# spotify/basic-pitch

Hardware: NVIDIA H100
Metric: audio_seconds_per_second (higher is better)
Workload: dtype f32

## Files before the change

basic_pitch_b200/_lib.py:

```python
from __future__ import annotations

import ctypes as C
import os
import pathlib
from typing import Optional

LIB_PATH = pathlib.Path(__file__).resolve().parent / "libbp_b200.so"

BP_OK = 0
BP_E_INVALID = -1
BP_E_CUDA = -2
BP_E_CAPACITY = -3
BP_E_NOMEM = -4

EXPORTS = [
    "bp_version", "bp_last_error", "bp_default_decode_params", "bp_num_windows", "bp_num_frames",
    "bp_model_create", "bp_model_destroy", "bp_model_device", "bp_model_param_block", "bp_model_refresh",
    "bp_model_launch_count", "bp_forward_device", "bp_forward_host", "bp_run_inference_device",
    "bp_run_inference_host", "bp_decode_device", "bp_decode_host", "bp_transcribe_host", "bp_transcribe_device",
    "bp_infer_onsets_host", "bp_pitch_bends_host", "bp_debug_activation", "bp_model_chunk_windows", "bp_model_set_path", "bp_model_profile", "bp_model_profile_read", "bp_debug_tc_plan", "bp_debug_tc_gather", "bp_debug_tc_gather_packed", "bp_debug_tc_b2", "bp_debug_tc_clocks", "bp_transcribe_files_host", "bp_host_alloc", "bp_host_free", "bp_last_required", "bp_resampled_length", "bp_load_pcm_device", "bp_load_pcm_host", "bp_debug_resample_filter", "bp_write_note_files", "bp_sonify_notes_host", "bp_load_pcm_files_device", "bp_transcribe_pcm_files_host", "bp_debug_pcm_layout", "bp_debug_frontend", "bp_model_set_debug_frontend", "bp_debug_chain_layout", "bp_debug_split_layout", "bp_decode_grid_device", "bp_decode_grid_host", "bp_decode_grid_chunk_params", "bp_default_score_params", "bp_frame_times", "bp_score_grid_device", "bp_score_grid_host", "bp_score_notes_host", "bp_multipitch_map", "bp_score_frames_grid_device", "bp_score_frames_grid_host", "bp_score_multipitch_host", "bp_score_salience_grid_device", "bp_score_salience_grid_host", "bp_score_salience_chunk_params", "bp_match_grid_device", "bp_match_grid_host", "bp_match_notes_host", "bp_score_onset_offset_grid_device", "bp_score_onset_offset_grid_host", "bp_score_onset_offset_notes_host",
]


class DecodeParams(C.Structure):
    _fields_ = [
        ("onset_thresh", C.c_double),
        ("frame_thresh", C.c_double),
        ("min_note_len", C.c_int32),
        ("energy_tol", C.c_int32),
        ("infer_onsets", C.c_int32),
        ("melodia_trick", C.c_int32),
        ("include_pitch_bends", C.c_int32),
        ("min_pitch_idx", C.c_int32),
        ("max_pitch_idx", C.c_int32),
        ("reserved", C.c_int32),
    ]


class Notes(C.Structure):
    _fields_ = [
        ("note_capacity", C.c_int32),
        ("bend_capacity", C.c_int32),
        ("note_off", C.c_void_p),
        ("start_frame", C.c_void_p),
        ("end_frame", C.c_void_p),
        ("pitch_midi", C.c_void_p),
        ("amplitude", C.c_void_p),
        ("bend_off", C.c_void_p),
        ("bends", C.c_void_p),
    ]


class NoteSet(C.Structure):
# ... 109 lines not shown
    lib.bp_match_notes_host.argtypes = [vp, C.POINTER(NoteSet), C.POINTER(NoteSet), i32, C.POINTER(ScoreParams), vp]
    lib.bp_score_onset_offset_grid_device.argtypes = [vp, vp, vp, vp, i32, C.POINTER(DecodeParams), i32,
                                                      C.POINTER(NoteSet), C.POINTER(ScoreParams), vp, vp, vp]
    lib.bp_score_onset_offset_grid_host.argtypes = [vp, vp, vp, vp, i32, C.POINTER(DecodeParams), i32,
                                                    C.POINTER(NoteSet), C.POINTER(ScoreParams), vp, vp]
    lib.bp_score_onset_offset_notes_host.argtypes = [vp, C.POINTER(NoteSet), C.POINTER(NoteSet), i32,
                                                     C.POINTER(ScoreParams), vp]
    lib.bp_multipitch_map.argtypes = [vp, i64, vp, i64, vp]
    lib.bp_score_frames_grid_device.argtypes = [vp, vp, vp, vp, i32, C.POINTER(DecodeParams), i32, C.POINTER(MultipitchSet),
                                                C.c_double, vp, vp, vp, vp]
    lib.bp_score_frames_grid_host.argtypes = [vp, vp, vp, vp, i32, C.POINTER(DecodeParams), i32, C.POINTER(MultipitchSet),
                                              C.c_double, vp, vp, vp]
    lib.bp_score_multipitch_host.argtypes = [vp, C.POINTER(MultipitchSet), C.POINTER(MultipitchSet), i32, C.c_double, vp]
    lib.bp_score_salience_grid_device.argtypes = [vp, vp, i32, vp, i32, C.POINTER(SalienceParams), i32,
                                                  C.POINTER(MultipitchSet), C.c_double, vp, vp, vp, vp]
    lib.bp_score_salience_grid_host.argtypes = [vp, vp, i32, vp, i32, C.POINTER(SalienceParams), i32,
                                                C.POINTER(MultipitchSet), C.c_double, vp, vp, vp]
    lib.bp_score_salience_chunk_params.argtypes = [i64, i64]
    lib.bp_score_salience_chunk_params.restype = i64
    lib.bp_transcribe_host.argtypes = [vp, vp, vp, i32, C.POINTER(DecodeParams), vp, vp, vp, vp, C.POINTER(Notes)]
    lib.bp_transcribe_device.argtypes = [vp, vp, vp, i32, C.POINTER(DecodeParams), vp, C.POINTER(Notes), vp]
    lib.bp_infer_onsets_host.argtypes = [vp, vp, vp, i64, vp]
    lib.bp_pitch_bends_host.argtypes = [vp, vp, i64, i32, vp, vp, vp, vp, vp, i64]
    lib.bp_debug_activation.argtypes = [vp, C.c_int, vp, i64]
    lib.bp_debug_frontend.argtypes = [vp, C.c_int, vp, i64]
    lib.bp_model_set_debug_frontend.argtypes = [vp, C.c_int]
    lib.bp_debug_chain_layout.argtypes = [vp, vp, vp]
    lib.bp_debug_split_layout.argtypes = [vp, vp]
    lib.bp_debug_tc_plan.argtypes = [C.c_int, vp, vp, vp, vp, vp, vp, vp]
    lib.bp_debug_tc_gather.argtypes = [C.c_int, vp, vp, vp, vp, vp]
    lib.bp_debug_tc_gather_packed.argtypes = [C.c_int, vp, vp, vp, vp]
    lib.bp_debug_tc_b2.argtypes = [C.c_int, vp, vp, vp]
    lib.bp_debug_tc_clocks.argtypes = [vp, C.c_int, vp, C.c_int]
    lib.bp_transcribe_files_host.argtypes = [vp, vp, vp, i32, C.POINTER(DecodeParams), vp, vp, vp, vp, C.POINTER(Notes)]
    lib.bp_host_alloc.argtypes = [sz]
    lib.bp_host_alloc.restype = vp
    lib.bp_host_free.argtypes = [vp]
    lib.bp_host_free.restype = None
    lib.bp_last_required.argtypes = [vp, vp]
    lib.bp_last_required.restype = None
    lib.bp_resampled_length.argtypes = [i64, i32]
    lib.bp_resampled_length.restype = i64
    lib.bp_load_pcm_device.argtypes = [vp, vp, i32, i64, i32, i32, vp, vp]
    lib.bp_load_pcm_host.argtypes = [vp, vp, i32, i64, i32, i32, vp]
    lib.bp_load_pcm_files_device.argtypes = [vp, C.POINTER(PcmFile), i32, vp, vp, vp]
    lib.bp_transcribe_pcm_files_host.argtypes = [vp, C.POINTER(PcmFile), i32, C.POINTER(DecodeParams), vp, vp, vp, vp, vp,
                                                 C.POINTER(Notes)]
    lib.bp_debug_pcm_layout.argtypes = [C.POINTER(PcmFile), i32, vp, vp]
    lib.bp_debug_resample_filter.argtypes = [i32, i32, vp, i64]
    lib.bp_debug_resample_filter.restype = i64
    lib.bp_write_note_files.argtypes = [i32, vp, vp, vp, vp, vp, vp, vp, vp, vp, i32, C.c_double, i32]
    lib.bp_sonify_notes_host.argtypes = [vp, i32, vp, vp, vp, vp, vp, vp, vp, i32, i32, vp, vp, i64]
    lib.bp_model_profile.argtypes = [vp, C.c_int]
    lib.bp_model_profile_read.argtypes = [vp, C.POINTER(C.c_double), C.POINTER(i64), C.POINTER(i64)]
    for name in EXPORTS:
        fn = getattr(lib, name)
        if fn.restype is C.c_int and name not in ("bp_version", "bp_model_device"):
            fn.errcheck = _check
    _lib = lib
    return lib


def _check(result, func, args):
    if result != BP_OK:
        raise BpError(result, load().bp_last_error().decode(errors="replace"))
    return result
# ... 1 lines not shown
```

basic_pitch_b200/csrc/api.cu:

```cuda
#include <cuda_runtime.h>

#include <algorithm>
#include <atomic>
#include <chrono>
#include <climits>
#include <cmath>
#include <cstdio>
#include <cstring>
#include <memory>
#include <thread>
#include <string>
#include <vector>

#include "bp_b200.h"
#include "kernels.cuh"

using namespace bp;

namespace {

thread_local std::string g_err;

int fail(int code, const std::string& msg) {
  g_err = msg;
// ... 2865 lines not shown
  sizes[0] = g.K_packed;
  if (b1) {
    std::vector<uint16_t> m;
    tc_build_b1(which, w, m);
    std::memcpy(b1, m.data(), m.size() * 2);
  }
  if (kmap) std::copy(g.kmap.begin(), g.kmap.end(), kmap);
  return BP_OK;
}

int bp_debug_tc_b2(int which, const float* w2, int32_t* sizes, uint16_t* tiles) {
  if (!w2 || !sizes || which < 0 || which > 2) return fail(BP_E_INVALID, "bp_debug_tc_b2: bad argument");
  std::vector<uint16_t> t;
  tc_build_b2(which, w2, t);
  const TcConvSpec sp = tc_spec(which);
  sizes[0] = sp.n2_tiles;
  sizes[1] = sp.n2;
  sizes[2] = sp.KH2;
  sizes[3] = sp.width;
  sizes[4] = sp.js;
  if (tiles) std::memcpy(tiles, t.data(), t.size() * 2);
  return BP_OK;
}

int bp_debug_tc_clocks(bp_model_t* m, int which, uint64_t* cycles, int reset) {
  if (!m || !cycles || which < 0 || which > 2) return fail(BP_E_INVALID, "bp_debug_tc_clocks: bad argument");
  DeviceGuard g(m->device);
  CK(cudaDeviceSynchronize());
  if (tc_read_clocks(which, reinterpret_cast<unsigned long long*>(cycles), reset != 0) != 0)
    return fail(BP_E_INVALID, "bp_debug_tc_clocks: the library was built without -DBP_TC_CLOCKS");
  return BP_OK;
}

int bp_model_profile(bp_model_t* m, int which) {
  if (!m) return fail(BP_E_INVALID, "bp_model_profile: null model");
  if (which < -1 || which > 6) return fail(BP_E_INVALID, "bp_model_profile: unknown kernel family");
  m->profile_which = which;
  m->prof_used = 0;
  m->prof_windows = 0;
  return BP_OK;
}

int bp_model_profile_read(bp_model_t* m, double* total_ms, int64_t* n_intervals, int64_t* n_windows) {
  if (!m || !total_ms || !n_intervals || !n_windows) return fail(BP_E_INVALID, "bp_model_profile_read: null argument");
  DeviceGuard g(m->device);
  CK(cudaDeviceSynchronize());
  double total = 0.0;
  for (size_t i = 0; i + 1 < m->prof_used; i += 2) {
    float ms = 0.f;
    CK(cudaEventElapsedTime(&ms, m->prof_ev[i], m->prof_ev[i + 1]));
    total += ms;
  }
  *total_ms = total;
  *n_intervals = (int64_t)(m->prof_used / 2);
  *n_windows = m->prof_windows;
  return BP_OK;
}

int bp_debug_activation(bp_model_t* m, int which, float* h_out, int64_t n_windows) {
  if (!m || !h_out) return fail(BP_E_INVALID, "bp_debug_activation: null argument");
  if (n_windows <= 0 || n_windows > m->chunk || n_windows > m->last_forward_n)
    return fail(BP_E_INVALID, "bp_debug_activation: only valid for the windows of a single-chunk forward call");
  DeviceGuard g(m->device);
  const float* src = nullptr;
  size_t per = 0;
  switch (which) {
// ... 101 lines not shown
```

basic_pitch_b200/csrc/kernels.cuh:

```cuda
#pragma once
#include <cuda_bf16.h>

#include <cstring>
#include <vector>

#include "common.cuh"

namespace bp {

void hcqt_setup();
constexpr int kLp2 = kTaps + 14;
struct Lowpass2 {
  float2 t[kLp2];
};
Lowpass2 lowpass_pairs(const float* h_lp );
void launch_decimate(const Lowpass2& lp, const float* audio, const WinDesc* desc, float* chain, int stage, int n_windows,
                     cudaStream_t st);
void launch_cqt(const float* audio, const WinDesc* desc, const float* chain, const float* wt, const float* scale,
                float* logmag, unsigned int* minmax, int n_windows, cudaStream_t st);
void launch_lognorm(float* y, const unsigned int* minmax, const float* bn , int n_windows,
                    cudaStream_t st);

struct CnnWeights {
  const float *contour1_wT, *contour1_b;
// ... 22 lines not shown
  int layer;
  int KH2, HALO, G0;
  int PD;
  int n2_tiles, n2, js, width, pass;
  int W;
  int slot[24];
  __host__ __device__ constexpr int n_ft() const { return (WOUT + FLT - 1) / FLT; }
  __host__ __device__ constexpr int tile_bins() const { return 8 * (chunks8 - 1); }
  __host__ __device__ constexpr int ksteps() const { return (KH * n_ci * W + 15) / 16; }
  __host__ __device__ constexpr int edge_per_side() const { return 2 * HALO + (layer == 0 ? 8 - HALO : 0); }
};
__host__ __device__ constexpr TcConvSpec tc_spec(int layer) {
  return layer == 0 ? TcConvSpec{3, 39, 1, 1, 19, 8, 16, 264, 8, {-36, 0, 36, 57, 72, 84, 93, 101}, kCqtBins,     40, 174, 3, 0, 5, 2, 9,  1,  1, 32, 5, 104, 40, 0, {}}
       : layer == 1 ? TcConvSpec{5, 5, 3, 2, 1, 32, 4, 88, 8, {-36, 0, 36, 57, 72, 84, 93, 101},   kCqtBins,     40, 174, 3, 1, 3, 1, 12, 12, 2, 16, 4, 32, 32,   6,
                                 {9, 10, 21, 22, 14, 4, 2, 1, 16, 3, 6, 13, 5, 17, 18, 20, 19, 23, 7, 0, 8, 15, 12, 11}}
                    : TcConvSpec{7, 7, 3, 3, 2, 32, 4, 88, 1, {0, 0, 0, 0, 0, 0, 0, 0},           kContourBins, 34, 175, 6, 2, 7, 1, 12, 12, 2, 32, 8, 64, 64,   8, {}};
}
__host__ __device__ constexpr int tc_group_tile(const TcConvSpec& s, int g, int slot) {
  if (g < 0 || g >= s.G0) return -1;
  const int run = g / s.PD, i = g - run * s.PD, ft = 2 * s.PD * run + slot * s.PD + i;
  return ft < s.n_ft() ? ft : -1;
}
__host__ __device__ constexpr int tc_tile_group(const TcConvSpec& s, int ft) {
  const int run = ft / (2 * s.PD), r = ft - run * 2 * s.PD, slot = r / s.PD;
  return ((run * s.PD + r - slot * s.PD) << 1) | slot;
}
__host__ __device__ constexpr bool tc_starts_range(const TcConvSpec& s, int g, int slot, bool item_start) {
  const int ft = tc_group_tile(s, g, slot);
  return item_start || ft <= 0 || tc_group_tile(s, g - 1, slot) != ft - 1;
}
__host__ __device__ constexpr bool tc_ends_range(const TcConvSpec& s, int g, int slot, bool item_end) {
  return item_end || tc_group_tile(s, g + 1, slot) != tc_group_tile(s, g, slot) + 1;
}
__host__ __device__ constexpr bool tc_item_starts(const TcConvSpec& s, int n_split, int g) {
  const int q = (g * n_split + s.G0 - 1) / s.G0;
  return q < n_split && q * s.G0 / n_split == g;
}
__host__ __device__ constexpr bool tc_pairing_ok(const TcConvSpec& s) {
  for (int ft = 0; ft < s.n_ft(); ++ft) {
    int n = 0;
    for (int g = 0; g < s.G0; ++g)
      for (int slot = 0; slot < 2; ++slot) n += tc_group_tile(s, g, slot) == ft;
    const int gs = tc_tile_group(s, ft);
    if (n != 1 || tc_group_tile(s, gs >> 1, gs & 1) != ft) return false;
  }
  return true;
}
struct TcConvPlan {
  TcConvSpec spec{};
  std::vector<uint16_t> tiles;
  std::vector<int> tile_seq;
  std::vector<uint32_t> slot_words[2];
  std::vector<int> group_step_off;
  std::vector<int> group_ft;
  int n_tiles = 0, n_groups = 0, n_uses = 0;
  void build(const TcConvSpec& spec, const float* w );
};
struct TcConvDev {
  int layer;
  const uint16_t* tiles;
  const uint16_t* b1;
  const uint16_t* b2;
  float bias1[32];
  float bias2;
  float note_w[9];
};
int tc_upload_program(const TcConvPlan& contour_plan, cudaStream_t st);
void tc_build_b1(int layer, const float* w, std::vector<uint16_t>& out, bool window8 = false);
struct TcGatherGeom {
  int K, n_ci, KH, wout;
  int K_packed;
  std::vector<int> starts, ranges;
  std::vector<int> kmap;
};
TcGatherGeom tc_gather_geometry(int layer);
void tc_build_b2(int layer, const float* w2, std::vector<uint16_t>& out);
void tc_build_b2_full(int layer, const float* w2, std::vector<uint16_t>& out);
int tc_rows_total(int n_windows, int rows_per_window);
size_t tc_edge_floats(const TcConvSpec& spec, int n_windows);
int tc_setup();
int tc_read_clocks(int layer, unsigned long long* out, bool reset);
struct UnwrapDesc {
  long long dst_base;
  int rows;
  int pad;
};
void launch_lognorm_split(const float* y, const unsigned int* minmax, const float* bn, __nv_bfloat16* dst,
                          const TcConvSpec& spec, int n_windows, int rows_stride, cudaStream_t st);
struct TcOut {
  float* raw = nullptr;
  float* unwrapped = nullptr;
  long long frame_stride = 0;
  long long raw_rows = 0;
  const UnwrapDesc* ud = nullptr;
  const float* note_raw = nullptr;
  __nv_bfloat16* chl = nullptr;
  int chl_rows = 0, chl_chunks = 0, chl_rpw = 0, chl_lead = 0;
  float* edge = nullptr;
  float* act = nullptr;
};
void launch_conv_tc(const __nv_bfloat16* data, const TcConvDev& dev, const TcOut& out, int n_windows, int rows_stride,
                    int n_sms, cudaStream_t st, bool fuse_next = false);
void launch_contour2_tc(const float* c1_nhwc, const CnnWeights& w, float* contour, __nv_bfloat16* chl, int rows_total,
                        int n_windows, cudaStream_t st);

void build_cqt_tc_weights(const float* cqt_real, const float* cqt_imag, std::vector<uint16_t>& out);
void cqt_tc_setup();
void launch_cqt_tc(const float* audio, const WinDesc* desc, const float* chain, const uint16_t* wtc, const float* scale,
                   float* logmag, unsigned int* minmax, int n_windows, int n_sms, cudaStream_t st);

void launch_rows_to_pm(const float* rows, long long n_frames, int width, float* pm, long long stride, long long dst_frame0,
                       cudaStream_t st, const UnwrapDesc* ud = nullptr, int n_windows = 0);
void launch_rows_to_cm(const float* rows, long long n_frames, float* cm, long long stride, long long dst_frame0,
                       cudaStream_t st, const UnwrapDesc* ud = nullptr, int n_windows = 0);
void launch_pm_to_rows(const float* pm, long long stride, long long src_frame0, long long n_frames, int width, float* rows,
                       cudaStream_t st);
void launch_cm_to_rows(const float* cm, long long stride, long long src_frame0, long long n_frames, float* rows,
                       cudaStream_t st);

long long ingest_output_length(long long n_frames, int sample_rate);
std::vector<double> ingest_filter(int up, int down);
int launch_ingest(int device, const void* d_pcm, int format, long long n_frames, int channels, int sample_rate, float* d_out,
                  cudaStream_t st);
struct IngestFile {
  const void* pcm;
  const float* hp;
  float* out;
  long long n_in, n_out;
  int channels, format, up, down, half, taps, span, pad;
};
int ingest_geometry(int format, int channels, int sample_rate, IngestFile& f);
int ingest_taps(int device, IngestFile& f);
long long ingest_ctas(long long n_out);
int launch_ingest_batch(const IngestFile* d_files, const int* d_cta_off, int n_files, int n_ctas, int max_span,
                        cudaStream_t st);
// ... 143 lines not shown
```

basic_pitch_b200/csrc/tc_conv.cu:

```cuda
#include <cuda.h>
#include <cuda_bf16.h>

#include <algorithm>
#include <cstdlib>
#include <cstring>
#include <unordered_map>
#include <vector>

#include "kernels.cuh"
#include "tc_ptx.cuh"

namespace bp {

namespace tc {
constexpr int kMTile = 64;
constexpr int kTileBytes = 8192;
constexpr int kMaxSteps = 1024;
constexpr int kMaxGroups = 15;
static_assert(tc_spec(0).G0 <= kMaxGroups, "contour groups in constant memory");
static_assert(tc_pairing_ok(tc_spec(0)) && tc_pairing_ok(tc_spec(1)) && tc_pairing_ok(tc_spec(2)), "group -> tile map");
static_assert(tc_spec(0).n_ft() <= 2 * tc_spec(0).G0 && tc_spec(1).n_ft() <= 2 * tc_spec(1).G0 &&
                  tc_spec(2).n_ft() <= 2 * tc_spec(2).G0,
              "every tile has a place in the reference pairing of the summation order (TcConvPlan::build)");
constexpr int kConsumerWarps = 8;
// ... 377 lines not shown
      const float* p = y + ((size_t)b * kFrames + t) * kCqtBins;
      float raw[2][8];
#pragma unroll
      for (int h = 0; h < 2; ++h)
#pragma unroll
        for (int j = 0; j < 8; ++j) {
          const int bin = (qa + h * half) * 8 + j;
          raw[h][j] = bin < kCqtBins ? __ldg(p + bin) : 0.f;
        }
#pragma unroll
      for (int h = 0; h < 2; ++h)
#pragma unroll
        for (int j = 0; j < 8; ++j)
          if ((qa + h * half) * 8 + j < kCqtBins) {
            const float q = (mx == 0.f) ? 0.f : __fdiv_rn(__fsub_rn(raw[h][j], mn), mx);
            v[h][j] = __fadd_rn(__fmul_rn(q, bn_scale), bn_bias);
          }
    }
  }
  const size_t plane = (size_t)chunks8 * rows_total * 8;
  store_split8(v[0], dst, ((size_t)qa * rows_total + d) * 8, plane);
  store_split8(v[1], dst, ((size_t)(qa + half) * rows_total + d) * 8, plane);
}

struct TcArgs {
  CUtensorMap data_map;
  int use_tmap;
  const __nv_bfloat16* data;
  const uint16_t* tiles;
  const uint16_t* b1;
  const uint16_t* b2;
  TcOut o;
  int edge_rows;
  int rows_total, n_mtiles, n_windows;
  int n_split;
  int row0;
  int chunks8;
  int ms, h2;
  float bias1[32], bias2, note_w[9];
};

__device__ __forceinline__ float sigmoidf_fast(float x) { return __fdividef(1.f, 1.f + __expf(-x)); }

namespace tc {
enum TcClk {
  kClkFull,
  kClkMma,
  kClkEpi,
  kClkData,
  kClkConsOther,
  kClkEmpty,
  kClkDataEmpty,
  kClkProdOther,
  kNumClk
};
}
#ifdef BP_TC_CLOCKS
__device__ unsigned long long g_tc_clocks[3][tc::kNumClk];
struct TcClocks {
  uint32_t t, c[tc::kNumClk];
  __device__ __forceinline__ TcClocks() {
    t = (uint32_t)clock();
#pragma unroll
    for (int k = 0; k < tc::kNumClk; ++k) c[k] = 0;
  }
  __device__ __forceinline__ void lap(int k) {
    const uint32_t n = (uint32_t)clock();
    c[k] += n - t;
    t = n;
  }
  __device__ __forceinline__ void flush(int layer) {
    if ((threadIdx.x & 31) == 0)
#pragma unroll
      for (int k = 0; k < tc::kNumClk; ++k) atomicAdd(&g_tc_clocks[layer][k], (unsigned long long)c[k]);
  }
};
#else
struct TcClocks {
  __device__ __forceinline__ void lap(int) {}
  __device__ __forceinline__ void flush(int) {}
};
#endif

int tc_read_clocks(int layer, unsigned long long* out, bool reset) {
#ifdef BP_TC_CLOCKS
  if (layer < 0 || layer > 2) return -1;
  if (cudaMemcpyFromSymbol(out, g_tc_clocks, tc::kNumClk * sizeof(unsigned long long),
                           (size_t)layer * tc::kNumClk * sizeof(unsigned long long)) != cudaSuccess)
    return -1;
  if (reset) {
    static const unsigned long long zero[tc::kNumClk] = {};
    if (cudaMemcpyToSymbol(g_tc_clocks, zero, sizeof(zero), (size_t)layer * sizeof(zero)) != cudaSuccess) return -1;
  }
  return 0;
#else
  (void)layer, (void)out, (void)reset;
  return -1;
#endif
}

__device__ __forceinline__ void slot_barrier(int slot) {
  asm volatile("bar.sync %0, 128;" ::"r"(1 + slot) : "memory");
}


struct RowOut {
  float* raw;
  float* unw;
  __nv_bfloat16* chl;
  float* edge;
  const float* note_col;
  int t;
  bool ok;
};

// ... 261 lines not shown
  unsigned char* s_data = smem;
  unsigned char* s_w = smem + SM.data_bytes;
  unsigned char* s_b1 = s_w + kStages * kTileBytes;
  unsigned char* s_b2 = s_b1 + SM.b1_bytes;
  float* s_p = reinterpret_cast<float*>(s_b2 + SM.b2_bytes);
  uint64_t* bars = reinterpret_cast<uint64_t*>(reinterpret_cast<unsigned char*>(s_p) + SM.p_bytes);
  uint64_t* full_w = bars;
  uint64_t* empty_w = bars + kStages;
  uint64_t* data_full = bars + 2 * kStages;
  uint64_t* data_empty = data_full + 1;
  uint64_t* b2_full = data_empty + 1;
  uint64_t* b1_full = b2_full + 1;
  uint32_t* issued = reinterpret_cast<uint32_t*>(b1_full + 1);

  const int warp = __shfl_sync(0xffffffffu, (int)(threadIdx.x >> 5), 0);
  const int lane = threadIdx.x & 31;
  constexpr uint32_t lbo = kDataRows * 16u;
  constexpr uint32_t plane_bytes = (L.chunks8 - 1) * lbo;

  if (threadIdx.x == 0) {
    for (int s = 0; s < kStages; ++s) {
      mbar_init(full_w + s, 1);
      mbar_init(empty_w + s, kConsumerWarps);
    }
    mbar_init(data_full, 1);
    mbar_init(data_empty, kConsumerWarps);
    mbar_init(b2_full, 1);
    mbar_init(b1_full, 1);
    *issued = 0;
    asm volatile("fence.mbarrier_init.release.cluster;" ::: "memory");
  }
  __syncthreads();

  const int n_items = a.n_mtiles * a.n_split;
  TcClocks clk;

  if (warp >= kConsumerWarps) {
    setmaxnreg_dec<kProducerRegs>();
    if (warp != kProducerWarp) return;
    const uint32_t leader = elect_one() ? 1u : 0u;
    if constexpr (kFused) bulk_g2s_expect_pred(s_b2, a.b2, (uint32_t)SM.b2_bytes, b2_full, leader);
    if constexpr (kGather) bulk_g2s_expect_pred(s_b1, a.b1, (uint32_t)SM.b1_bytes, b1_full, leader);
    uint32_t stage = 0, ph_w = 0, ph_d = 0, n_fill = 0;
    const size_t plane_elems = (size_t)L.chunks8 * a.rows_total * 8;
    for (int it = blockIdx.x; it < n_items; it += gridDim.x) {
      const int mt = it / a.n_split, sp = it % a.n_split;
      const int g0 = sp * L.G0 / a.n_split, g1 = (sp + 1) * L.G0 / a.n_split;
      clk.lap(kClkProdOther);
      mbar_wait_wd(data_empty, ph_d ^ 1, 1);
      clk.lap(kClkDataEmpty);
      const size_t row = (size_t)mt * a.ms + a.row0;
      if (leader) {
        mbar_expect_tx(data_full, 2 * plane_bytes);
        if (a.use_tmap) {
          tma_load_4d(s_data, &a.data_map, 0, (int)row, 0, 0, data_full);
        } else {
          for (int p = 0; p < 2; ++p)
            for (int c = 0; c < a.chunks8 - 1; ++c)
              bulk_g2s(s_data + p * plane_bytes + c * lbo, a.data + p * plane_elems + ((size_t)c * a.rows_total + row) * 8,
                       lbo, data_full);
        }
      }
      __syncwarp();
      ph_d ^= 1;
      if constexpr (kGather) continue;
      const int s0 = c_group_step_off[g0], s1 = c_group_step_off[g1];
      int tile = c_tile_seq[s0];
      for (int s = s0; s < s1; ++s) {
        const int tile_next = c_tile_seq[s + 1];
        clk.lap(kClkProdOther);
        mbar_wait_wd(empty_w + stage, ph_w ^ 1, 2);
        clk.lap(kClkEmpty);
        bulk_g2s_expect_pred(s_w + stage * kTileBytes, a.tiles + (size_t)tile * (kTileBytes / 2), kTileBytes, full_w + stage,
                             leader);
        const bool skip = c_prog[0][s] == kNoUse || c_prog[1][s] == kNoUse;
        mbar_arrive_cnt_pred(empty_w + stage, kConsumerWarps / 2, skip ? leader : 0u);
        counter_publish(issued, ++n_fill);
        if (++stage == kStages) {
          stage = 0;
          ph_w ^= 1;
        }
        tile = tile_next;
      }
    }
    clk.lap(kClkProdOther);
    clk.flush(LAYER);
  } else {
    setmaxnreg_inc<kConsumerRegs>();
    const int slot = warp >> 2, wq = warp & 3, gq = lane >> 2, qd = lane & 3;
    const int tid = threadIdx.x & 127;
    const int fr0 = 16 * wq + gq;
    uint32_t stage = 0, ph_w = 0, ph_d = 0, n_fill = 0;
    const uint32_t a_hi = smem_u32(s_data), a_lo = a_hi + plane_bytes, w_base = smem_u32(s_w);
    const uint32_t* prog = c_prog[slot];
    float* sp_rows = s_p + slot * 64 * PS;
    if constexpr (kFused) mbar_wait_wd(b2_full, 0, 6);
    if constexpr (kGather) mbar_wait_wd(b1_full, 0, 7);
    for (int it = blockIdx.x; it < n_items; it += gridDim.x) {
      const int mt = it / a.n_split, spl = it % a.n_split;
      const int g0 = spl * L.G0 / a.n_split, g1 = (spl + 1) * L.G0 / a.n_split;
      bool live[2];
      int rb[2], rt[2];
#pragma unroll
      for (int rr = 0; rr < 2; ++rr) {
        const int m = mt * a.ms - a.h2 + fr0 + 8 * rr;
        rb[rr] = m >= 0 ? m / L.rows_per_window : 0;
        rt[rr] = m - rb[rr] * L.rows_per_window;
        live[rr] = m >= 0 && (rb[rr] < a.n_windows) && (rt[rr] < kFrames);
      }
      RowOut ro{};
      float carry[4] = {0.f, 0.f, 0.f, 0.f};
      float hold[6] = {0.f, 0.f, 0.f, 0.f, 0.f, 0.f};
      if constexpr (kFused) {
        const int row = tid;
        const int q = mt * a.ms - 2 * a.h2 + row;
        const int b = q >= 0 ? q / L.rows_per_window : 0, t = q - b * L.rows_per_window;
        ro.ok = row < 64 && row >= 2 * a.h2 && q >= 0 && b < a.n_windows && t < kFrames;
        ro.t = t;
        if (ro.ok) {
          ro.edge = a.o.edge + q;
          int uf = -1;
          if (a.o.ud) {
            const UnwrapDesc u = a.o.ud[b];
            const int tt = t - kOverlapHalf;
            if ((unsigned)tt < (unsigned)max(u.rows, 0)) uf = (int)(u.dst_base + tt);
          }
          if constexpr (LAYER == 0) {
            ro.chl = a.o.chl + ((size_t)a.o.chl_lead + (size_t)b * a.o.chl_rpw + t) * 8;
            if (a.o.raw) ro.raw = a.o.raw + ((size_t)b * kFrames + t) * 8;
            if (uf >= 0) ro.unw = a.o.unwrapped + (size_t)uf * 8;
          } else {
            if (a.o.raw) ro.raw = a.o.raw + (size_t)b * kFrames + t;
            if (uf >= 0) ro.unw = a.o.unwrapped + uf;
// ... 114 lines not shown
                float* d = sp_rows + (fr0 + 8 * rr) * PS + 8 * i - q * PC + 2 * qd;
                d[0] = p[4 * i + 2 * rr];
                d[1] = p[4 * i + 2 * rr + 1];
              }
            }
            slot_barrier(slot);
            if (tid < 64) {
#pragma unroll
              for (int j = q * JP; j < NJ && j < (q + 1) * JP; ++j) {
                float s = 0.f;
#pragma unroll
                for (int ta = 0; ta < KH2; ++ta)
                  if (tid - ta >= 0) s += sp_rows[(tid - ta) * PS + j * JS - q * PC + (KH2 - 1 - ta)];
                S[j] = s;
              }
            }
          }
          if (tid < 64) {
            if constexpr (LAYER == 0) {
              finish_contour_tile(a, ro, S, ft, first, last, carry, hold);
            } else {
              float c2[2] = {carry[0], carry[1]};
              finish_pitch_tile<LAYER>(a, ro, S, c2, ft, first, last);
              carry[0] = c2[0];
              carry[1] = c2[1];
            }
          }
        }
        clk.lap(kClkEpi);
      }
    }
    clk.lap(kClkConsOther);
    clk.flush(LAYER);
  }
}


struct EdgeFixArgs {
  TcOut o;
  int edge_rows, n_rows;
  uint32_t edges;
  int n_windows;
  float bias2, note_w[9];
};

__host__ __device__ constexpr uint32_t tc_edge_mask(const TcConvSpec& s, int n_split) {
  uint32_t m = 0;
  for (int b = 1; b < s.n_ft(); ++b) {
    const int gs = tc_tile_group(s, b);
    if (tc_starts_range(s, gs >> 1, gs & 1, tc_item_starts(s, n_split, gs >> 1))) m |= 1u << b;
  }
  return m;
}
static_assert(tc_spec(0).n_ft() <= 32 && tc_spec(1).n_ft() <= 32 && tc_spec(2).n_ft() <= 32, "boundary mask");
static_assert(tc_edge_mask(tc_spec(0), 1) == 0x1fffeu && tc_edge_mask(tc_spec(1), 1) == 1u << 12,
              "contour: every tile a range of its own; onset: the slot boundary only");

template <int LAYER>
constexpr int kEdgeThreads = LAYER == 0 ? 1 : 2 * tc_spec(LAYER).HALO;

template <int LAYER>
__device__ __forceinline__ void edge_fix_boundary(const EdgeFixArgs& a, int ft_b, int R, int b, int t, int uf, int k) {
  constexpr TcConvSpec L = tc_spec(LAYER);
  const int e = ft_b - 1;
  if constexpr (LAYER == 0) {
    const float* lo = a.o.edge + (size_t)(e * 2 + 0) * L.edge_per_side() * a.edge_rows + R;
    const float* hi = a.o.edge + (size_t)(e * 2 + 1) * L.edge_per_side() * a.edge_rows + R;
    float fx[4];
#pragma unroll
    for (int q = 0; q < 4; ++q)
      fx[q] = sigmoidf_fast((lo[(size_t)q * a.edge_rows] + hi[(size_t)q * a.edge_rows]) + a.bias2);
    float va[8], vb[8];
#pragma unroll
    for (int q = 0; q < 6; ++q) {
      va[q] = hi[(size_t)(4 + q) * a.edge_rows];
      vb[2 + q] = lo[(size_t)(4 + q) * a.edge_rows];
    }
    va[6] = fx[0], va[7] = fx[1], vb[0] = fx[2], vb[1] = fx[3];
    __nv_bfloat16* chl = a.o.chl + ((size_t)a.o.chl_lead + (size_t)b * a.o.chl_rpw + t) * 8;
    const size_t plane = (size_t)a.o.chl_chunks * a.o.chl_rows * 8;
#pragma unroll
    for (int c = 0; c < 2; ++c) {
      const int chunk = 2 * ft_b - 1 + c;
      const float(&v)[8] = c ? vb : va;
      store_split8(v, chl, (size_t)chunk * a.o.chl_rows * 8, plane);
      const float4 x0 = make_float4(v[0], v[1], v[2], v[3]), x1 = make_float4(v[4], v[5], v[6], v[7]);
      if (a.o.raw) {
        float4* d = reinterpret_cast<float4*>(a.o.raw + ((size_t)chunk * a.o.raw_rows + (size_t)b * kFrames + t) * 8);
        d[0] = x0, d[1] = x1;
// ... 9 lines not shown
  if (f < 0 || f >= L.WOUT) return;
  float x = (a.o.edge[((size_t)(e * 2 + 0) * L.edge_per_side() + k) * a.edge_rows + R] +
             a.o.edge[((size_t)(e * 2 + 1) * L.edge_per_side() + k) * a.edge_rows + R]) + a.bias2;
  if (a.o.note_raw) {
#pragma unroll
    for (int dt = 0; dt < 3; ++dt)
#pragma unroll
      for (int df = 0; df < 3; ++df) {
        const int tt = t + dt - 1, ff = f + df - 1;
        if ((unsigned)tt < (unsigned)kFrames && (unsigned)ff < (unsigned)kPitches)
          x = fmaf(__ldg(a.o.note_raw + (size_t)ff * a.o.raw_rows + (size_t)b * kFrames + tt), a.note_w[dt * 3 + df], x);
      }
  }
  const float v = sigmoidf_fast(x);
  if (a.o.raw) a.o.raw[(size_t)f * a.o.raw_rows + (size_t)b * kFrames + t] = v;
  if (uf >= 0) a.o.unwrapped[(size_t)f * a.o.frame_stride + uf] = v;
}

template <int LAYER>
__global__ void edge_fix_kernel(const EdgeFixArgs a) {
  constexpr TcConvSpec L = tc_spec(LAYER);
  const long long idx = (long long)blockIdx.x * blockDim.x + threadIdx.x;
  if (idx >= (long long)a.n_rows * kEdgeThreads<LAYER>) return;
  const int R = (int)(idx % a.n_rows);
  const int k = (int)(idx / a.n_rows);
  const int b = R / L.rows_per_window, t = R - b * L.rows_per_window;
  if (b >= a.n_windows || t >= kFrames) return;
  int uf = -1;
  if (a.o.ud) {
    const UnwrapDesc u = a.o.ud[b];
    const int tt = t - kOverlapHalf;
    if ((unsigned)tt < (unsigned)max(u.rows, 0)) uf = (int)(u.dst_base + tt);
  }
  for (uint32_t m = a.edges; m; m &= m - 1) edge_fix_boundary<LAYER>(a, __ffs(m) - 1, R, b, t, uf, k);
}
int tc_rows_total(int n_windows, int rows_per_window) {
  return n_windows * rows_per_window + tc::kMTile + 16;
}

int tc_setup() {
  using namespace tc;
  cudaError_t e = cudaFuncSetAttribute(conv_tc_kernel<0, false>, cudaFuncAttributeMaxDynamicSharedMemorySize, tc_smem(0, false).total());
  if (e == cudaSuccess) e = cudaFuncSetAttribute(conv_tc_kernel<1, true>, cudaFuncAttributeMaxDynamicSharedMemorySize, tc_smem(1, true).total());
  if (e == cudaSuccess) e = cudaFuncSetAttribute(conv_tc_kernel<2, true>, cudaFuncAttributeMaxDynamicSharedMemorySize, tc_smem(2, true).total());
  if (e == cudaSuccess) e = cudaFuncSetAttribute(conv_tc_kernel<0, true>, cudaFuncAttributeMaxDynamicSharedMemorySize, tc_smem(0, true).total());
  return e == cudaSuccess ? 0 : -1;
}

void launch_lognorm_split(const float* y, const unsigned int* minmax, const float* bn, __nv_bfloat16* dst,
                          const TcConvSpec& sp, int n_windows, int rows_stride, cudaStream_t st) {
  const int rows_used = tc_rows_total(n_windows, sp.rows_per_window);
  const long long cells = (long long)rows_used * (sp.chunks8 / 2);
  lognorm_split_kernel<<<(unsigned)((cells + 255) / 256), 256, 0, st>>>(y, minmax, bn, dst, n_windows, rows_used, rows_stride,
                                                                       sp.chunks8, sp.rows_per_window, sp.lead_rows);
}

size_t tc_edge_floats(const TcConvSpec& sp, int n_windows) {
  const int ms = tc::kMTile - (sp.KH2 - 1);
  const int n_mtiles = (n_windows * sp.rows_per_window + ms - 1) / ms;
  return (size_t)(sp.n_ft() - 1) * 2 * sp.edge_per_side() * ((size_t)n_mtiles * ms);
}

template <int LAYER, bool FUSED>
static void launch_layer(const TcArgs& a, const EdgeFixArgs& ef, int grid, cudaStream_t st) {
  conv_tc_kernel<LAYER, FUSED><<<grid, tc::kThreads, tc::tc_smem(LAYER, FUSED).total(), st>>>(a);
  if (FUSED) {
    const long long total = (long long)ef.n_rows * kEdgeThreads<LAYER>;
    edge_fix_kernel<LAYER><<<(unsigned)((total + 255) / 256), 256, 0, st>>>(ef);
  }
}

void launch_conv_tc(const __nv_bfloat16* data, const TcConvDev& dev, const TcOut& o, int n_windows, int rows_stride,
                    int n_sms, cudaStream_t st, bool fuse_next) {
  const TcConvSpec sp = tc_spec(dev.layer);
  const bool fused = dev.layer != 0 || fuse_next;
  TcArgs a{};
  a.data = data;
  a.tiles = dev.tiles;
  a.b1 = dev.b1;
  a.b2 = dev.b2;
  a.o = o;
  a.rows_total = rows_stride;
  a.h2 = fused ? (sp.KH2 - 1) / 2 : 0;
  a.ms = tc::kMTile - 2 * a.h2;
  a.n_mtiles = (n_windows * sp.rows_per_window + a.ms - 1) / a.ms;
  a.edge_rows = a.n_mtiles * a.ms;
  a.n_windows = n_windows;
  int split = 1;
  double best = 1e30;
  for (int s = 1; s <= sp.G0; ++s) {
    const int waves = (a.n_mtiles * s + n_sms - 1) / n_sms;
    const double cost = waves * ((sp.G0 + s - 1) / s + 0.5);
    if (cost < best - 1e-9) best = cost, split = s;
  }
  a.n_split = split;
  a.row0 = sp.lead_rows - sp.PT - a.h2;
  a.chunks8 = sp.chunks8;
  std::copy_n(dev.bias1, 32, a.bias1);
  a.bias2 = dev.bias2;
  std::copy_n(dev.note_w, 9, a.note_w);
  const int n_items = a.n_mtiles * a.n_split;
  const int grid = n_items < n_sms ? n_items : n_sms;
  {
    using EncodeFn = CUresult (*)(CUtensorMap*, CUtensorMapDataType, cuuint32_t, void*, const cuuint64_t*, const cuuint64_t*,
                                  const cuuint32_t*, const cuuint32_t*, CUtensorMapInterleave, CUtensorMapSwizzle,
                                  CUtensorMapL2promotion, CUtensorMapFloatOOBfill);
    static EncodeFn encode = [] {
      void* fn = nullptr;
      cudaDriverEntryPointQueryResult q;
      if (cudaGetDriverEntryPoint("cuTensorMapEncodeTiled", &fn, cudaEnableDefault, &q) != cudaSuccess ||
          q != cudaDriverEntryPointSuccess)
        fn = nullptr;
      return reinterpret_cast<EncodeFn>(fn);
    }();
    a.use_tmap = 0;
    static const bool want_tmap = getenv("BP_B200_TMAP") != nullptr;
    if (encode && want_tmap) {
      const cuuint64_t dims[4] = {8, (cuuint64_t)rows_stride, (cuuint64_t)sp.chunks8, 2};
      const cuuint64_t strides[3] = {16, (cuuint64_t)rows_stride * 16, (cuuint64_t)sp.chunks8 * rows_stride * 16};
      const cuuint32_t box[4] = {8, (cuuint32_t)(tc::kMTile + sp.KH - 1), (cuuint32_t)(sp.chunks8 - 1), 2};
      const cuuint32_t estr[4] = {1, 1, 1, 1};
      if (encode(&a.data_map, CU_TENSOR_MAP_DATA_TYPE_BFLOAT16, 4, const_cast<__nv_bfloat16*>(data), dims, strides, box, estr,
                 CU_TENSOR_MAP_INTERLEAVE_NONE, CU_TENSOR_MAP_SWIZZLE_NONE, CU_TENSOR_MAP_L2_PROMOTION_L2_128B,
                 CU_TENSOR_MAP_FLOAT_OOB_FILL_NONE) == CUDA_SUCCESS)
        a.use_tmap = 1;
    }
  }
  EdgeFixArgs ef{};
  ef.o = o;
  ef.edge_rows = a.edge_rows;
  ef.n_rows = n_windows * sp.rows_per_window;
  ef.edges = tc_edge_mask(sp, split);
  ef.n_windows = n_windows;
  ef.bias2 = dev.bias2;
  std::copy_n(dev.note_w, 9, ef.note_w);
  if (dev.layer == 1)
    launch_layer<1, true>(a, ef, grid, st);
  else if (dev.layer == 2)
    launch_layer<2, true>(a, ef, grid, st);
  else if (fuse_next)
    launch_layer<0, true>(a, ef, grid, st);
  else
    launch_layer<0, false>(a, ef, grid, st);
}

}
```

include/bp_b200.h:

```cpp
#ifndef BP_B200_H
#define BP_B200_H

#include <stddef.h>
#include <stdint.h>

#ifdef __cplusplus
extern "C" {
#endif

#define BP_OK 0
#define BP_E_INVALID (-1)
#define BP_E_CUDA (-2)
#define BP_E_CAPACITY (-3)
#define BP_E_NOMEM (-4)

#define BP_SAMPLE_RATE 22050
#define BP_WINDOW_SAMPLES 43844
#define BP_WINDOW_FRAMES 172
#define BP_N_PITCHES 88
#define BP_N_CONTOUR_BINS 264
#define BP_OVERLAP_FRAMES 30
#define BP_HOP_SAMPLES 36164
#define BP_HOP_FRAMES 142
#define BP_LEAD_ZEROS 3840
// ... 186 lines not shown
  int32_t sample_format;
  int32_t channels;
  int32_t sample_rate;
  int32_t reserved;
} bp_pcm_file_t;

int bp_load_pcm_files_device(bp_model_t* m, const bp_pcm_file_t* files, int32_t n_files, float* d_audio,
                             int64_t* h_sample_off, void* stream);
int bp_transcribe_pcm_files_host(bp_model_t* m, const bp_pcm_file_t* files, int32_t n_files,
                                 const bp_decode_params_t* params, float* h_note, float* h_onset, float* h_contour,
                                 int64_t* h_frame_off, int64_t* h_sample_off, bp_notes_t* notes);
int bp_debug_pcm_layout(const bp_pcm_file_t* files, int32_t n_files, int64_t* byte_off, int64_t* sample_off);

int bp_write_note_files(int32_t n_files, const char* const* midi_paths, const char* const* csv_paths,
                        const int32_t* note_off, const double* start_s, const double* end_s, const int32_t* pitch_midi,
                        const float* amplitude, const int32_t* bend_off, const int32_t* bends,
                        int32_t multiple_pitch_bends, double midi_tempo, int32_t n_threads);

int bp_sonify_notes_host(bp_model_t* m, int32_t n_files, const int32_t* note_off, const double* start_s,
                         const double* end_s, const int32_t* pitch_midi, const float* amplitude, const int32_t* bend_off,
                         const int32_t* bends, int32_t multiple_pitch_bends, int32_t sample_rate, int64_t* h_sample_off,
                         double* h_audio, int64_t capacity);

int64_t bp_debug_resample_filter(int32_t up, int32_t down, double* taps, int64_t capacity);

int bp_debug_tc_plan(int which, const float* w, int32_t* sizes, uint16_t* tiles, int32_t* tile_seq, uint32_t* slot_words,
                     int32_t* group_step_off, int32_t* group_ft);

int bp_debug_tc_gather(int which, const float* w, int32_t* sizes, uint16_t* b1, int32_t* starts, int32_t* ranges);
int bp_debug_tc_gather_packed(int which, const float* w, int32_t* sizes, uint16_t* b1, int32_t* kmap);

int bp_debug_tc_b2(int which, const float* w2, int32_t* sizes, uint16_t* tiles);

int bp_model_profile(bp_model_t* m, int which);
int bp_model_profile_read(bp_model_t* m, double* total_ms, int64_t* n_intervals, int64_t* n_windows);

int bp_debug_tc_clocks(bp_model_t* m, int which, uint64_t* cycles, int reset);

#ifdef __cplusplus
}
#endif
#endif
```

Baseline: 148,000.

## Schedule tensor-core conv work as whole M-tiles plus cost-balanced split tail

Replaces the uniform per-M-tile group split with a schedule in which full waves of M-tiles run unsplit and only the tail M-tiles are split into group ranges. The ranges are chosen by a min-max partition over estimated per-group costs, so the last partial wave is load-balanced across SMs. Edge-fix masks now differ between the full and tail regions. This aims to remove the redundant split overhead in full waves and the imbalance in the last wave, but depends on the heuristic cost model being accurate. It also adds debug hooks for per-CTA busy timing.

Result: faster. 156,400, median of 6 (+5.7%).

```diff
diff --git a/basic_pitch_b200/_lib.py b/basic_pitch_b200/_lib.py
--- a/basic_pitch_b200/_lib.py
+++ b/basic_pitch_b200/_lib.py
@@ -18,7 +18,7 @@
     "bp_model_create", "bp_model_destroy", "bp_model_device", "bp_model_param_block", "bp_model_refresh",
     "bp_model_launch_count", "bp_forward_device", "bp_forward_host", "bp_run_inference_device",
     "bp_run_inference_host", "bp_decode_device", "bp_decode_host", "bp_transcribe_host", "bp_transcribe_device",
-    "bp_infer_onsets_host", "bp_pitch_bends_host", "bp_debug_activation", "bp_model_chunk_windows", "bp_model_set_path", "bp_model_profile", "bp_model_profile_read", "bp_debug_tc_plan", "bp_debug_tc_gather", "bp_debug_tc_gather_packed", "bp_debug_tc_b2", "bp_debug_tc_clocks", "bp_transcribe_files_host", "bp_host_alloc", "bp_host_free", "bp_last_required", "bp_resampled_length", "bp_load_pcm_device", "bp_load_pcm_host", "bp_debug_resample_filter", "bp_write_note_files", "bp_sonify_notes_host", "bp_load_pcm_files_device", "bp_transcribe_pcm_files_host", "bp_debug_pcm_layout", "bp_debug_frontend", "bp_model_set_debug_frontend", "bp_debug_chain_layout", "bp_debug_split_layout", "bp_decode_grid_device", "bp_decode_grid_host", "bp_decode_grid_chunk_params", "bp_default_score_params", "bp_frame_times", "bp_score_grid_device", "bp_score_grid_host", "bp_score_notes_host", "bp_multipitch_map", "bp_score_frames_grid_device", "bp_score_frames_grid_host", "bp_score_multipitch_host", "bp_score_salience_grid_device", "bp_score_salience_grid_host", "bp_score_salience_chunk_params", "bp_match_grid_device", "bp_match_grid_host", "bp_match_notes_host", "bp_score_onset_offset_grid_device", "bp_score_onset_offset_grid_host", "bp_score_onset_offset_notes_host",
+    "bp_infer_onsets_host", "bp_pitch_bends_host", "bp_debug_activation", "bp_model_chunk_windows", "bp_model_set_path", "bp_model_profile", "bp_model_profile_read", "bp_debug_tc_plan", "bp_debug_tc_gather", "bp_debug_tc_gather_packed", "bp_debug_tc_b2", "bp_debug_tc_schedule", "bp_debug_tc_clocks", "bp_debug_tc_cta_busy", "bp_transcribe_files_host", "bp_host_alloc", "bp_host_free", "bp_last_required", "bp_resampled_length", "bp_load_pcm_device", "bp_load_pcm_host", "bp_debug_resample_filter", "bp_write_note_files", "bp_sonify_notes_host", "bp_load_pcm_files_device", "bp_transcribe_pcm_files_host", "bp_debug_pcm_layout", "bp_debug_frontend", "bp_model_set_debug_frontend", "bp_debug_chain_layout", "bp_debug_split_layout", "bp_decode_grid_device", "bp_decode_grid_host", "bp_decode_grid_chunk_params", "bp_default_score_params", "bp_frame_times", "bp_score_grid_device", "bp_score_grid_host", "bp_score_notes_host", "bp_multipitch_map", "bp_score_frames_grid_device", "bp_score_frames_grid_host", "bp_score_multipitch_host", "bp_score_salience_grid_device", "bp_score_salience_grid_host", "bp_score_salience_chunk_params", "bp_match_grid_device", "bp_match_grid_host", "bp_match_notes_host", "bp_score_onset_offset_grid_device", "bp_score_onset_offset_grid_host", "bp_score_onset_offset_notes_host",
 ]
 
 
@@ -194,6 +194,8 @@
     lib.bp_debug_tc_gather_packed.argtypes = [C.c_int, vp, vp, vp, vp]
     lib.bp_debug_tc_b2.argtypes = [C.c_int, vp, vp, vp]
     lib.bp_debug_tc_clocks.argtypes = [vp, C.c_int, vp, C.c_int]
+    lib.bp_debug_tc_schedule.argtypes = [C.c_int, C.c_int, C.c_int, C.c_int, vp, vp, vp]
+    lib.bp_debug_tc_cta_busy.argtypes = [vp, C.c_int, vp, C.c_int, C.c_int]
     lib.bp_transcribe_files_host.argtypes = [vp, vp, vp, i32, C.POINTER(DecodeParams), vp, vp, vp, vp, C.POINTER(Notes)]
     lib.bp_host_alloc.argtypes = [sz]
     lib.bp_host_alloc.restype = vp
diff --git a/basic_pitch_b200/csrc/api.cu b/basic_pitch_b200/csrc/api.cu
--- a/basic_pitch_b200/csrc/api.cu
+++ b/basic_pitch_b200/csrc/api.cu
@@ -2921,6 +2921,39 @@
   return BP_OK;
 }
 
+int bp_debug_tc_schedule(int which, int fused, int n_windows, int n_sms, int32_t* sizes, int32_t* items, uint32_t* edges) {
+  if (!sizes || which < 0 || which > 2 || n_windows < 1 || n_sms < 1)
+    return fail(BP_E_INVALID, "bp_debug_tc_schedule: bad argument");
+  const TcConvSpec sp = tc_spec(which);
+  int ms = 0;
+  const TcSchedule s = tc_schedule(which, fused != 0 || which != 0, n_windows, n_sms, &ms);
+  sizes[0] = s.n_items();
+  sizes[1] = s.grid;
+  sizes[2] = s.n_mtiles;
+  sizes[3] = s.n_full;
+  sizes[4] = s.n_ranges;
+  sizes[5] = ms;
+  sizes[6] = s.n_full * ms;
+  sizes[7] = sp.G0;
+  if (items)
+    for (int it = 0; it < s.n_items(); ++it) s.item(it, sp.G0, items[3 * it], items[3 * it + 1], items[3 * it + 2]);
+  if (edges) {
+    edges[0] = tc_edge_mask(sp, 1u);
+    edges[1] = tc_edge_mask(sp, s.tail_starts());
+  }
+  return BP_OK;
+}
+
+int bp_debug_tc_cta_busy(bp_model_t* m, int which, uint64_t* ns, int n, int reset) {
+  if (!m || (!ns && n) || which < 0 || which > 2 || n < 0 || n > kTcMaxCtas)
+    return fail(BP_E_INVALID, "bp_debug_tc_cta_busy: bad argument");
+  DeviceGuard g(m->device);
+  CK(cudaDeviceSynchronize());
+  if (tc_read_busy(which, reinterpret_cast<unsigned long long*>(ns), n, reset != 0) != 0)
+    return fail(BP_E_INVALID, "bp_debug_tc_cta_busy: the library was built without -DBP_TC_CLOCKS");
+  return BP_OK;
+}
+
 int bp_model_profile(bp_model_t* m, int which) {
   if (!m) return fail(BP_E_INVALID, "bp_model_profile: null model");
   if (which < -1 || which > 6) return fail(BP_E_INVALID, "bp_model_profile: unknown kernel family");
diff --git a/basic_pitch_b200/csrc/kernels.cuh b/basic_pitch_b200/csrc/kernels.cuh
--- a/basic_pitch_b200/csrc/kernels.cuh
+++ b/basic_pitch_b200/csrc/kernels.cuh
@@ -78,9 +78,31 @@
 __host__ __device__ constexpr bool tc_ends_range(const TcConvSpec& s, int g, int slot, bool item_end) {
   return item_end || tc_group_tile(s, g + 1, slot) != tc_group_tile(s, g, slot) + 1;
 }
-__host__ __device__ constexpr bool tc_item_starts(const TcConvSpec& s, int n_split, int g) {
-  const int q = (g * n_split + s.G0 - 1) / s.G0;
-  return q < n_split && q * s.G0 / n_split == g;
+struct TcSchedule {
+  int n_mtiles, n_full, n_tail, n_ranges, grid;
+  unsigned char bounds[16];
+  __host__ __device__ int n_items() const { return n_full + n_tail * n_ranges; }
+  __host__ __device__ uint32_t tail_starts() const {
+    uint32_t m = 0;
+    for (int q = 0; q < n_ranges; ++q) m |= 1u << bounds[q];
+    return m;
+  }
+  __host__ __device__ void item(int it, int G0, int& mt, int& g0, int& g1) const {
+    if (it < n_full) {
+      mt = it, g0 = 0, g1 = G0;
+      return;
+    }
+    const int j = it - n_full, q = j / n_tail;
+    mt = n_full + (j - q * n_tail), g0 = bounds[q], g1 = bounds[q + 1];
+  }
+};
+__host__ __device__ constexpr uint32_t tc_edge_mask(const TcConvSpec& s, uint32_t starts) {
+  uint32_t m = 0;
+  for (int b = 1; b < s.n_ft(); ++b) {
+    const int gs = tc_tile_group(s, b);
+    if (tc_starts_range(s, gs >> 1, gs & 1, (starts >> (gs >> 1)) & 1u)) m |= 1u << b;
+  }
+  return m;
 }
 __host__ __device__ constexpr bool tc_pairing_ok(const TcConvSpec& s) {
   for (int ft = 0; ft < s.n_ft(); ++ft) {
@@ -126,6 +148,8 @@
 size_t tc_edge_floats(const TcConvSpec& spec, int n_windows);
 int tc_setup();
 int tc_read_clocks(int layer, unsigned long long* out, bool reset);
+constexpr int kTcMaxCtas = 256;
+int tc_read_busy(int layer, unsigned long long* out, int n, bool reset);
 struct UnwrapDesc {
   long long dst_base;
   int rows;
@@ -147,6 +171,7 @@
 };
 void launch_conv_tc(const __nv_bfloat16* data, const TcConvDev& dev, const TcOut& out, int n_windows, int rows_stride,
                     int n_sms, cudaStream_t st, bool fuse_next = false);
+TcSchedule tc_schedule(int layer, bool fused, int n_windows, int n_sms, int* ms = nullptr);
 void launch_contour2_tc(const float* c1_nhwc, const CnnWeights& w, float* contour, __nv_bfloat16* chl, int rows_total,
                         int n_windows, cudaStream_t st);
 
diff --git a/basic_pitch_b200/csrc/tc_conv.cu b/basic_pitch_b200/csrc/tc_conv.cu
--- a/basic_pitch_b200/csrc/tc_conv.cu
+++ b/basic_pitch_b200/csrc/tc_conv.cu
@@ -433,8 +433,8 @@
   const uint16_t* b2;
   TcOut o;
   int edge_rows;
-  int rows_total, n_mtiles, n_windows;
-  int n_split;
+  int rows_total, n_windows;
+  TcSchedule sch;
   int row0;
   int chunks8;
   int ms, h2;
@@ -458,12 +458,24 @@
 }
 #ifdef BP_TC_CLOCKS
 __device__ unsigned long long g_tc_clocks[3][tc::kNumClk];
+__device__ unsigned long long g_tc_busy[3][kTcMaxCtas];
+__device__ __forceinline__ unsigned long long globaltimer_ns() {
+  unsigned long long t;
+  asm volatile("mov.u64 %0, %globaltimer;" : "=l"(t));
+  return t;
+}
 struct TcClocks {
   uint32_t t, c[tc::kNumClk];
+  unsigned long long t0;
   __device__ __forceinline__ TcClocks() {
     t = (uint32_t)clock();
+    t0 = globaltimer_ns();
 #pragma unroll
     for (int k = 0; k < tc::kNumClk; ++k) c[k] = 0;
+  }
+  __device__ __forceinline__ void cta_end(int layer) {
+    asm volatile("bar.sync 3, 256;" ::: "memory");
+    if (threadIdx.x == 0 && blockIdx.x < kTcMaxCtas) atomicAdd(&g_tc_busy[layer][blockIdx.x], globaltimer_ns() - t0);
   }
   __device__ __forceinline__ void lap(int k) {
     const uint32_t n = (uint32_t)clock();
@@ -480,8 +492,25 @@
 struct TcClocks {
   __device__ __forceinline__ void lap(int) {}
   __device__ __forceinline__ void flush(int) {}
+  __device__ __forceinline__ void cta_end(int) {}
 };
 #endif
+
+int tc_read_busy(int layer, unsigned long long* out, int n, bool reset) {
+#ifdef BP_TC_CLOCKS
+  if (layer < 0 || layer > 2 || n < 0 || n > kTcMaxCtas) return -1;
+  const size_t row = kTcMaxCtas * sizeof(unsigned long long);
+  if (n && cudaMemcpyFromSymbol(out, g_tc_busy, n * sizeof(unsigned long long), (size_t)layer * row) != cudaSuccess) return -1;
+  if (reset) {
+    static const unsigned long long zero[kTcMaxCtas] = {};
+    if (cudaMemcpyToSymbol(g_tc_busy, zero, row, (size_t)layer * row) != cudaSuccess) return -1;
+  }
+  return 0;
+#else
+  (void)layer, (void)out, (void)n, (void)reset;
+  return -1;
+#endif
+}
 
 int tc_read_clocks(int layer, unsigned long long* out, bool reset) {
 #ifdef BP_TC_CLOCKS
@@ -809,7 +838,7 @@
   }
   __syncthreads();
 
-  const int n_items = a.n_mtiles * a.n_split;
+  const int n_items = a.sch.n_items();
   TcClocks clk;
 
   if (warp >= kConsumerWarps) {
@@ -821,8 +850,8 @@
     uint32_t stage = 0, ph_w = 0, ph_d = 0, n_fill = 0;
     const size_t plane_elems = (size_t)L.chunks8 * a.rows_total * 8;
     for (int it = blockIdx.x; it < n_items; it += gridDim.x) {
-      const int mt = it / a.n_split, sp = it % a.n_split;
-      const int g0 = sp * L.G0 / a.n_split, g1 = (sp + 1) * L.G0 / a.n_split;
+      int mt, g0, g1;
+      a.sch.item(it, L.G0, mt, g0, g1);
       clk.lap(kClkProdOther);
       mbar_wait_wd(data_empty, ph_d ^ 1, 1);
       clk.lap(kClkDataEmpty);
@@ -874,8 +903,8 @@
     if constexpr (kFused) mbar_wait_wd(b2_full, 0, 6);
     if constexpr (kGather) mbar_wait_wd(b1_full, 0, 7);
     for (int it = blockIdx.x; it < n_items; it += gridDim.x) {
-      const int mt = it / a.n_split, spl = it % a.n_split;
-      const int g0 = spl * L.G0 / a.n_split, g1 = (spl + 1) * L.G0 / a.n_split;
+      int mt, g0, g1;
+      a.sch.item(it, L.G0, mt, g0, g1);
       bool live[2];
       int rb[2], rt[2];
 #pragma unroll
@@ -1056,6 +1085,7 @@
     }
     clk.lap(kClkConsOther);
     clk.flush(LAYER);
+    clk.cta_end(LAYER);
   }
 }
 
@@ -1063,22 +1093,16 @@
 struct EdgeFixArgs {
   TcOut o;
   int edge_rows, n_rows;
-  uint32_t edges;
+  uint32_t edges_full, edges_tail;
+  int tail_row0;
   int n_windows;
   float bias2, note_w[9];
 };
 
-__host__ __device__ constexpr uint32_t tc_edge_mask(const TcConvSpec& s, int n_split) {
-  uint32_t m = 0;
-  for (int b = 1; b < s.n_ft(); ++b) {
-    const int gs = tc_tile_group(s, b);
-    if (tc_starts_range(s, gs >> 1, gs & 1, tc_item_starts(s, n_split, gs >> 1))) m |= 1u << b;
-  }
-  return m;
-}
 static_assert(tc_spec(0).n_ft() <= 32 && tc_spec(1).n_ft() <= 32 && tc_spec(2).n_ft() <= 32, "boundary mask");
-static_assert(tc_edge_mask(tc_spec(0), 1) == 0x1fffeu && tc_edge_mask(tc_spec(1), 1) == 1u << 12,
-              "contour: every tile a range of its own; onset: the slot boundary only");
+static_assert(tc_edge_mask(tc_spec(0), 1u) == 0x1fffeu && tc_edge_mask(tc_spec(1), 1u) == 1u << 12 &&
+                  tc_edge_mask(tc_spec(2), 1u) == 1u << 12,
+              "whole M-tiles: contour: every tile a range of its own; onset / note: the slot boundary only");
 
 template <int LAYER>
 constexpr int kEdgeThreads = LAYER == 0 ? 1 : 2 * tc_spec(LAYER).HALO;
@@ -1154,7 +1178,8 @@
     const int tt = t - kOverlapHalf;
     if ((unsigned)tt < (unsigned)max(u.rows, 0)) uf = (int)(u.dst_base + tt);
   }
-  for (uint32_t m = a.edges; m; m &= m - 1) edge_fix_boundary<LAYER>(a, __ffs(m) - 1, R, b, t, uf, k);
+  for (uint32_t m = R < a.tail_row0 ? a.edges_full : a.edges_tail; m; m &= m - 1)
+    edge_fix_boundary<LAYER>(a, __ffs(m) - 1, R, b, t, uf, k);
 }
 int tc_rows_total(int n_windows, int rows_per_window) {
   return n_windows * rows_per_window + tc::kMTile + 16;
@@ -1181,6 +1206,81 @@
   const int ms = tc::kMTile - (sp.KH2 - 1);
   const int n_mtiles = (n_windows * sp.rows_per_window + ms - 1) / ms;
   return (size_t)(sp.n_ft() - 1) * 2 * sp.edge_per_side() * ((size_t)n_mtiles * ms);
+}
+
+namespace tc {
+constexpr double kEpiUses = 14.0, kItemUsesContour = 20.0, kItemTilesPitch = 0.25;
+}
+static void tc_group_costs(int layer, std::vector<double>& cost, double& item) {
+  using namespace tc;
+  const TcConvSpec sp = tc_spec(layer);
+  cost.assign(sp.G0, 0.0);
+  for (int g = 0; g < sp.G0; ++g)
+    for (int sl = 0; sl < 2; ++sl) cost[g] += tc_group_tile(sp, g, sl) >= 0 ? (layer == 0 ? kEpiUses : 1.0) : 0.0;
+  item = layer == 0 ? kItemUsesContour : kItemTilesPitch;
+  if (layer != 0) return;
+  static const std::vector<double> uses = [] {
+    const TcConvSpec s = tc_spec(0);
+    std::vector<float> w((size_t)s.COUT * s.n_ci * s.KH * s.KW, 0.f);
+    TcConvPlan pl;
+    pl.build(s, w.data());
+    std::vector<double> u(s.G0, 0.0);
+    for (int g = 0; g < s.G0; ++g)
+      for (int st = pl.group_step_off[g]; st < pl.group_step_off[g + 1]; ++st)
+        for (int sl = 0; sl < 2; ++sl) u[g] += pl.slot_words[sl][st] != kNoUse ? 1.0 : 0.0;
+    return u;
+  }();
+  for (int g = 0; g < sp.G0; ++g) cost[g] += uses[g];
+}
+
+TcSchedule tc_schedule(int layer, bool fused, int n_windows, int n_sms, int* ms_out) {
+  const TcConvSpec sp = tc_spec(layer);
+  const int h2 = fused || layer != 0 ? (sp.KH2 - 1) / 2 : 0;
+  const int ms = tc::kMTile - 2 * h2;
+  if (ms_out) *ms_out = ms;
+  std::vector<double> cost;
+  double item;
+  tc_group_costs(layer, cost, item);
+  const int G = sp.G0;
+  std::vector<double> pre(G + 1, 0.0);
+  for (int g = 0; g < G; ++g) pre[g + 1] = pre[g] + cost[g];
+  TcSchedule s{};
+  s.n_mtiles = (n_windows * sp.rows_per_window + ms - 1) / ms;
+  s.n_full = s.n_mtiles / n_sms * n_sms;
+  s.n_tail = s.n_mtiles - s.n_full;
+  s.n_ranges = 1;
+  s.bounds[0] = 0, s.bounds[1] = (unsigned char)G;
+  if (s.n_tail > 0) {
+    std::vector<std::vector<double>> best(G + 1, std::vector<double>(G + 1, 1e300));
+    std::vector<std::vector<int>> cut(G + 1, std::vector<int>(G + 1, G));
+    for (int g = 0; g < G; ++g) best[1][g] = pre[G] - pre[g];
+    for (int r = 2; r <= G; ++r)
+      for (int g = 0; g + r <= G; ++g)
+        for (int e = g + 1; e + r - 1 <= G; ++e) {
+          const double v = std::max(pre[e] - pre[g], best[r - 1][e]);
+          if (v < best[r][g]) best[r][g] = v, cut[r][g] = e;
+        }
+    double best_t = 1e300;
+    for (int r = 1; r <= G; ++r) {
+      unsigned char b[16];
+      b[0] = 0;
+      for (int q = 0; q < r; ++q) b[q + 1] = (unsigned char)(q + 1 < r ? cut[r - q][b[q]] : G);
+      const int n_items = s.n_tail * r, grid = s.n_full ? n_sms : std::min(n_items, n_sms);
+      double worst = 0.0;
+      for (int c = 0; c < grid && c < n_items; ++c) {
+        double t = 0.0;
+        for (int j = c; j < n_items; j += grid) t += pre[b[j / s.n_tail + 1]] - pre[b[j / s.n_tail]] + item;
+        worst = std::max(worst, t);
+      }
+      if (worst < best_t * (1.0 - 1e-9)) {
+        best_t = worst;
+        s.n_ranges = r;
+        std::copy_n(b, r + 1, s.bounds);
+      }
+    }
+  }
+  s.grid = std::min(s.n_items(), n_sms);
+  return s;
 }
 
 template <int LAYER, bool FUSED>
@@ -1204,25 +1304,15 @@
   a.o = o;
   a.rows_total = rows_stride;
   a.h2 = fused ? (sp.KH2 - 1) / 2 : 0;
-  a.ms = tc::kMTile - 2 * a.h2;
-  a.n_mtiles = (n_windows * sp.rows_per_window + a.ms - 1) / a.ms;
-  a.edge_rows = a.n_mtiles * a.ms;
+  a.sch = tc_schedule(dev.layer, fused, n_windows, n_sms, &a.ms);
+  a.edge_rows = a.sch.n_mtiles * a.ms;
   a.n_windows = n_windows;
-  int split = 1;
-  double best = 1e30;
-  for (int s = 1; s <= sp.G0; ++s) {
-    const int waves = (a.n_mtiles * s + n_sms - 1) / n_sms;
-    const double cost = waves * ((sp.G0 + s - 1) / s + 0.5);
-    if (cost < best - 1e-9) best = cost, split = s;
-  }
-  a.n_split = split;
   a.row0 = sp.lead_rows - sp.PT - a.h2;
   a.chunks8 = sp.chunks8;
   std::copy_n(dev.bias1, 32, a.bias1);
   a.bias2 = dev.bias2;
   std::copy_n(dev.note_w, 9, a.note_w);
-  const int n_items = a.n_mtiles * a.n_split;
-  const int grid = n_items < n_sms ? n_items : n_sms;
+  const int grid = a.sch.grid;
   {
     using EncodeFn = CUresult (*)(CUtensorMap*, CUtensorMapDataType, cuuint32_t, void*, const cuuint64_t*, const cuuint64_t*,
                                   const cuuint32_t*, const cuuint32_t*, CUtensorMapInterleave, CUtensorMapSwizzle,
@@ -1252,7 +1342,9 @@
   ef.o = o;
   ef.edge_rows = a.edge_rows;
   ef.n_rows = n_windows * sp.rows_per_window;
-  ef.edges = tc_edge_mask(sp, split);
+  ef.edges_full = tc_edge_mask(sp, 1u);
+  ef.edges_tail = tc_edge_mask(sp, a.sch.tail_starts());
+  ef.tail_row0 = a.sch.n_full * a.ms;
   ef.n_windows = n_windows;
   ef.bias2 = dev.bias2;
   std::copy_n(dev.note_w, 9, ef.note_w);
diff --git a/include/bp_b200.h b/include/bp_b200.h
--- a/include/bp_b200.h
+++ b/include/bp_b200.h
@@ -242,10 +242,13 @@
 
 int bp_debug_tc_b2(int which, const float* w2, int32_t* sizes, uint16_t* tiles);
 
+int bp_debug_tc_schedule(int which, int fused, int n_windows, int n_sms, int32_t* sizes, int32_t* items, uint32_t* edges);
+
 int bp_model_profile(bp_model_t* m, int which);
 int bp_model_profile_read(bp_model_t* m, double* total_ms, int64_t* n_intervals, int64_t* n_windows);
 
 int bp_debug_tc_clocks(bp_model_t* m, int which, uint64_t* cycles, int reset);
+int bp_debug_tc_cta_busy(bp_model_t* m, int which, uint64_t* ns, int n, int reset);
 
 #ifdef __cplusplus
 }
```
